# SkyworkAI/Vitron

Measured on NVIDIA H100. Metric: Vicuna-7B generated tokens/s, batch-8 x (256 vision + 512 text) prefill + 128-token greedy decode, incl. ViT-L/14 encode, higher is better.
Workload: dtype bf16

## Files before the change

### include/vitron_b200.h

```cpp
#ifndef VITRON_B200_H_
#define VITRON_B200_H_

#include <stddef.h>
#include <stdint.h>

#ifdef __cplusplus
extern "C" {
#endif

#ifndef __CUDA_RUNTIME_H__
typedef struct CUstream_st* cudaStream_t;
#endif

#define VB_ACT_NONE 0
#define VB_ACT_GELU 1
#define VB_ACT_QUICK_GELU 2
#define VB_ACT_RELU 3
#define VB_ACT_SILU 4

#define VB_GLU_NONE 0
#define VB_GLU_SWIGLU 1
#define VB_GLU_GEGLU 2

typedef struct vb_epilogue {
  const void* bias;
  const void* rowbias;
  int64_t rowbias_rows;
  const void* residual;
  int64_t ldr;
  float alpha;
  int32_t act;
  int32_t glu;
  int32_t out_fp32;
  const float* rowscale;
  float rms_eps;
} vb_epilogue;

const char* vb200_version(void);
const char* vb200_last_error(void);
int vb200_device_ok(void);
int vb200_set_pdl(int enable);
int vb200_set_attention_impl(int impl);
int vb200_attention_watchdog(uint32_t* out3);
int vb200_attention_tc_occupancy(int head_dim);

size_t vb200_gemm_bf16_workspace_size(int64_t M, int64_t N, int64_t K);
int vb200_gemm_bf16(const void* A, int64_t lda, const void* W, int64_t ldw, void* out, int64_t ldo,
                    int64_t M, int64_t N, int64_t K, const vb_epilogue* epi, void* workspace,
                    size_t workspace_bytes, cudaStream_t stream);

int vb200_gemm_nf4(const void* A, int64_t lda, const void* codes, const void* scales, const float* kscale, void* out,
                   int64_t ldo, int64_t M, int64_t N, int64_t K, const vb_epilogue* epi, cudaStream_t stream);
int vb200_nf4_dequant(const void* codes, const void* scales, const float* kscale, void* out, int64_t N, int64_t K,
                      cudaStream_t stream);



size_t vb200_conv_nhwc_workspace_size(int64_t nb, int64_t h, int64_t w, int64_t cin, int64_t cout, int kh, int kw,
                                      int stride, int pad_h, int pad_w);
int vb200_conv_nhwc_bf16(const void* X, const void* Wt, void* out, int64_t nb, int64_t h,
                         int64_t w, int64_t cin, int64_t cout, int kh, int kw, int stride,
                         int pad_h, int pad_w, const vb_epilogue* epi, void* workspace,
                         size_t workspace_bytes, cudaStream_t stream);
int vb200_set_gemm_impl(int impl);
int vb200_set_gemm_debug(int resident_b, int dbg);

int vb200_conv_nhwc_direct(const void* X, const void* Wt, const void* bias, void* out, int64_t nb,
                           int64_t h, int64_t w, int64_t cin, int64_t cout, int kh, int kw,
                           int stride, int pad_h, int pad_w, cudaStream_t stream);

int vb200_rmsnorm(const void* x, int64_t ldx, const void* weight, void* out, int64_t ldo,
                  int64_t rows, int64_t d, float eps, cudaStream_t stream);
int vb200_row_rstd(const void* x, int64_t ldx, float* out, int64_t rows, int64_t d, float eps,
                   cudaStream_t stream);
int vb200_layernorm(const void* x, int64_t ldx, const void* weight, const void* bias, void* out,
                    int64_t ldo, int64_t rows, int64_t d, float eps, cudaStream_t stream);
size_t vb200_groupnorm_workspace_size(int64_t n, int64_t groups, int64_t c);
int vb200_groupnorm_nhwc(const void* x, const void* weight, const void* bias, void* out, int64_t n,
                         int64_t spatial, int64_t c, int64_t groups, float eps, int act,
                         void* workspace, size_t workspace_bytes, cudaStream_t stream);

int vb200_attention(const void* q, const void* k, const void* v, void* out, int64_t B, int64_t H,
                    int64_t Sq, int64_t Skv, int64_t head_dim, int64_t q_sb, int64_t q_ss,
                    int64_t q_sh, int64_t k_sb, int64_t k_ss, int64_t k_sh, int64_t v_sb,
                    int64_t v_ss, int64_t v_sh, int64_t o_sb, int64_t o_ss, int64_t o_sh,
                    float scale, int causal, const int32_t* kv_len, const uint8_t* mask,
                    int64_t m_sb, int64_t m_sh, int64_t m_sq, cudaStream_t stream);
size_t vb200_attention_workspace_size(int64_t B, int64_t H, int64_t Sq, int64_t Skv, int64_t head_dim, int causal);
// ... 138 lines not shown
```

### vitron_b200/_lib.py

```python
import ctypes as C
import os

_HERE = os.path.dirname(os.path.abspath(__file__))
LIB_PATH = os.path.join(_HERE, "libvitron_b200.so")

ACT_NONE, ACT_GELU, ACT_QUICK_GELU, ACT_RELU, ACT_SILU = 0, 1, 2, 3, 4
GLU_NONE, GLU_SWIGLU, GLU_GEGLU = 0, 1, 2

_ERR = {-1: "VB_ERR_ARG", -2: "VB_ERR_CUDA", -3: "VB_ERR_WORKSPACE", -4: "VB_ERR_UNSUPPORTED",
        -5: "VB_ERR_DRIVER"}


class Epilogue(C.Structure):
    _fields_ = [
        ("bias", C.c_void_p), ("rowbias", C.c_void_p), ("rowbias_rows", C.c_int64),
        ("residual", C.c_void_p), ("ldr", C.c_int64), ("alpha", C.c_float),
        ("act", C.c_int32), ("glu", C.c_int32), ("out_fp32", C.c_int32),
        ("rowscale", C.c_void_p), ("rms_eps", C.c_float),
    ]


_p, _i64, _i32, _f, _sz = C.c_void_p, C.c_int64, C.c_int, C.c_float, C.c_size_t

SIGNATURES = {
    "vb200_version": (C.c_char_p, []),
    "vb200_last_error": (C.c_char_p, []),
    "vb200_device_ok": (_i32, []),
    "vb200_set_pdl": (_i32, [_i32]),
    "vb200_set_attention_impl": (_i32, [_i32]),
    "vb200_attention_watchdog": (_i32, [_p]),
    "vb200_attention_tc_occupancy": (_i32, [_i32]),
    "vb200_gemm_bf16_workspace_size": (_sz, [_i64, _i64, _i64]),
    "vb200_gemm_bf16": (_i32, [_p, _i64, _p, _i64, _p, _i64, _i64, _i64, _i64, C.POINTER(Epilogue), _p, _sz, _p]),
    "vb200_gemm_nf4": (_i32, [_p, _i64, _p, _p, _p, _p, _i64, _i64, _i64, _i64, C.POINTER(Epilogue), _p]),
    "vb200_nf4_dequant": (_i32, [_p, _p, _p, _p, _i64, _i64, _p]),
    "vb200_conv_nhwc_workspace_size": (_sz, [_i64, _i64, _i64, _i64, _i64, _i32, _i32, _i32, _i32, _i32]),
    "vb200_conv_nhwc_bf16": (_i32, [_p, _p, _p, _i64, _i64, _i64, _i64, _i64, _i32, _i32, _i32, _i32, _i32,
                                    C.POINTER(Epilogue), _p, _sz, _p]),
    "vb200_set_gemm_impl": (_i32, [_i32]),
    "vb200_set_gemm_debug": (_i32, [_i32, _i32]),
    "vb200_conv_nhwc_direct": (_i32, [_p, _p, _p, _p, _i64, _i64, _i64, _i64, _i64, _i32, _i32, _i32, _i32, _i32, _p]),
    "vb200_rmsnorm": (_i32, [_p, _i64, _p, _p, _i64, _i64, _i64, _f, _p]),
    "vb200_row_rstd": (_i32, [_p, _i64, _p, _i64, _i64, _f, _p]),
    "vb200_layernorm": (_i32, [_p, _i64, _p, _p, _p, _i64, _i64, _i64, _f, _p]),
    "vb200_groupnorm_workspace_size": (_sz, [_i64, _i64, _i64]),
    "vb200_groupnorm_nhwc": (_i32, [_p, _p, _p, _p, _i64, _i64, _i64, _i64, _f, _i32, _p, _sz, _p]),
    "vb200_attention": (_i32, [_p, _p, _p, _p, _i64, _i64, _i64, _i64, _i64] + [_i64] * 12 +
                        [_f, _i32, _p, _p, _i64, _i64, _i64, _p]),
    "vb200_attention_workspace_size": (_sz, [_i64, _i64, _i64, _i64, _i64, _i32]),
    "vb200_attention_ws": (_i32, [_p, _p, _p, _p, _i64, _i64, _i64, _i64, _i64] + [_i64] * 12 +
                           [_f, _i32, _p, _p, _i64, _i64, _i64, _p, _sz, _p]),
    "vb200_attention_paged_workspace_size": (_sz, [_i64, _i64, _i64, _i64, _i64]),
    "vb200_attention_paged": (_i32, [_p, _i64, _i64, _i64, _p, _p, _i64, _p, _i64, _p, _p, _p, _i64, _i64, _i64,
                                     _i64, _i64, _i64, _i64, _i64, _i64, _f, _p, _sz, _p]),
    "vb200_attention_short": (_i32, [_p, _p, _p, _p, _i64, _i64, _i64, _i64] + [_i64] * 17 + [_f, _p]),
    "vb200_add_rowgroup": (_i32, [_p, _p, _p, _i64, _i64, _i64, _i64, _p]),
    "vb200_rope_kv_append": (_i32, [_p, _i64, _p, _p, _p, _p, _p, _p, _i64, _i64, _i64, _i64, _i64, _f, _p]),
    "vb200_attn_decode_workspace_size": (_sz, [_i64, _i64, _i64, _i64]),
    "vb200_attn_decode_paged": (_i32, [_p, _i64, _p, _p, _p, _i64, _p, _p, _i64, _i64, _i64, _i64, _i64, _i64,
                                       _f, _p, _sz, _p]),
    "vb200_rope_table": (_i32, [_p, _p, _i64, _i64, _f, _p]),
    "vb200_attn_decode_rope": (_i32, [_p, _i64, _p, _p, _p, _p, _i64, _p, _p, _i64, _i64, _i64, _i64, _i64, _i64,
                                      _f, _p, _sz, _p]),
    "vb200_attn_decode_rope_beam": (_i32, [_p, _i64, _p, _p, _p, _p, _i64, _p, _p, _i64, _p, _p, _i64, _i64, _i64, _i64,
                                           _i64, _i64, _f, _p, _sz, _p]),
    "vb200_splice_multimodal": (_i32, [_p, _i64, _p, _i64, _p, _p, _i64, _i64, _p]),
    "vb200_argmax_rows": (_i32, [_p, _i32, _i64, _i64, _i64, _p, _p]),
    "vb200_argmax_advance": (_i32, [_p, _i64, _i64, _i64, _p, _p, _p, _p, _p, _i64, _p, _p]),
    "vb200_sample_advance": (_i32, [_p, _i64, _i64, _i64, _p, _p, _p, _p, _p, _p, _i64, _p, _p]),
    "vb200_beam_workspace_size": (_sz, [_i64]),
    "vb200_beam_advance": (_i32, [_p, _i64, _i64, _i64, _i64, _p, _p, _p, _p, _p, _i64, _p, _p, _p, _p, _p, _i64, _p, _p,
# ... 53 lines not shown
```

### vitron_b200/csrc/gemv.cu

```cuda
#include "common.cuh"
#include "vitron_b200.h"
#include <type_traits>

namespace vb {

struct GemvParams {
  const bf16* W; long long ldw;
  const bf16* X; long long ldx;
  void* out; long long ldo;
  int M, N, K;
  const bf16* bias; const bf16* rowbias; int rowbias_rows;
  const bf16* residual; long long ldr;
  float alpha; int act, glu, out_fp32;
  const float* rowscale; float rms_eps;
};

__device__ __forceinline__ float gemv_act(float x, int act) {
  switch (act) {
    case VB_ACT_GELU: return gelu_erf(x);
    case VB_ACT_QUICK_GELU: return quick_gelu(x);
    case VB_ACT_RELU: return fmaxf(x, 0.f);
    case VB_ACT_SILU: return silu(x);
    default: return x;
  }
}

__device__ __forceinline__ void mma16816(float (&c)[4], uint32_t a0, uint32_t a1, uint32_t a2, uint32_t a3,
                                         uint32_t b0, uint32_t b1) {
  asm("mma.sync.aligned.m16n8k16.row.col.f32.bf16.bf16.f32 {%0,%1,%2,%3}, {%4,%5,%6,%7}, {%8,%9}, {%0,%1,%2,%3};"
      : "+f"(c[0]), "+f"(c[1]), "+f"(c[2]), "+f"(c[3])
      : "r"(a0), "r"(a1), "r"(a2), "r"(a3), "r"(b0), "r"(b1));
}

__device__ __forceinline__ uint4 ldg_stream(const bf16* p, bool ok) {
  uint4 v = make_uint4(0, 0, 0, 0);
  if (ok) asm volatile("ld.global.nc.L1::no_allocate.v4.u32 {%0,%1,%2,%3}, [%4];" : "=r"(v.x), "=r"(v.y), "=r"(v.z), "=r"(v.w) : "l"(p));
  return v;
}
__device__ __forceinline__ uint4 ldg_cached(const bf16* p, bool ok) {
  uint4 v = make_uint4(0, 0, 0, 0);
  if (ok) v = __ldg(reinterpret_cast<const uint4*>(p));
  return v;
}

template <int ROWS, int NT>
__global__ void __launch_bounds__(256, 2) gemv_bf16_kernel(const GemvParams p) {
  constexpr int WARPS = 8;
  constexpr int RG = ROWS / 16;
  constexpr int KS = WARPS / RG;
  constexpr int G = 2;
  __shared__ float red[2][WARPS][16][NT * 8 + 1];
  __shared__ float red_sq[WARPS][NT * 8];
  __shared__ float rstd_s[NT * 8];

  const int warp = threadIdx.x >> 5, lane = threadIdx.x & 31;
  const int g = lane >> 2, t = lane & 3;
  const int rg = warp % RG, ks = warp / RG;
  const int ntiles = (p.N + ROWS - 1) / ROWS;
  const bf16* x0 = p.X + static_cast<long long>(min(g, p.M - 1)) * p.ldx;
  const bf16* x1 = p.X + static_cast<long long>(min(g + 8, p.M - 1)) * p.ldx;
  const bool x0ok = g < p.M, x1ok = (NT == 2) && (g + 8 < p.M);

  const int chunks = (p.K + 63) / 64;
  const int base = chunks / KS, rem = chunks % KS;
  const int c0 = ks * base + min(ks, rem);
  const int c1 = c0 + base + (ks < rem ? 1 : 0);
  const int ngroups = (c1 - c0 + G - 1) / G;
  const int npairs = (ngroups + 1) / 2;

  const bool do_rms = p.rms_eps > 0.f && p.rowscale == nullptr;
  float sq0 = 0.f, sq1 = 0.f;

  struct Buf { uint4 wl[G][2], wh[G][2]; };
  auto load_group = [&](Buf& bf, int tile, int grp) {
    const int row0 = tile * ROWS + rg * 16;
    const bf16* wa = p.W + static_cast<long long>(min(row0 + g, p.N - 1)) * p.ldw;
    const bf16* wb = p.W + static_cast<long long>(min(row0 + g + 8, p.N - 1)) * p.ldw;
    const bool live = tile < ntiles;
#pragma unroll
    for (int u = 0; u < G; ++u) {
      const int c = c0 + grp * G + u;
      const int k0 = c * 64 + 8 * t, k1 = k0 + 32;
      const bool in = live && c < c1;
      const bool ok0 = in && k0 < p.K, ok1 = in && k1 < p.K;
      bf.wl[u][0] = ldg_stream(wa + k0, ok0); bf.wl[u][1] = ldg_stream(wa + k1, ok1);
      bf.wh[u][0] = ldg_stream(wb + k0, ok0); bf.wh[u][1] = ldg_stream(wb + k1, ok1);
    }
  };
  float acc[NT][4];
  auto compute_group = [&](const Buf& bf, int grp, bool first_tile) {
    uint4 xa[G][2], xb[G][2];
#pragma unroll
    for (int u = 0; u < G; ++u) {
      const int c = c0 + grp * G + u;
      const int k0 = c * 64 + 8 * t, k1 = k0 + 32;
      const bool in = c < c1;
      const bool ok0 = in && k0 < p.K, ok1 = in && k1 < p.K;
      xa[u][0] = ldg_cached(x0 + k0, ok0 && x0ok); xa[u][1] = ldg_cached(x0 + k1, ok1 && x0ok);
      if (NT == 2) { xb[u][0] = ldg_cached(x1 + k0, ok0 && x1ok); xb[u][1] = ldg_cached(x1 + k1, ok1 && x1ok); }
    }
#pragma unroll
    for (int u = 0; u < G; ++u) {
      const uint32_t al[8] = {bf.wl[u][0].x, bf.wl[u][0].y, bf.wl[u][0].z, bf.wl[u][0].w, bf.wl[u][1].x, bf.wl[u][1].y, bf.wl[u][1].z, bf.wl[u][1].w};
      const uint32_t ah[8] = {bf.wh[u][0].x, bf.wh[u][0].y, bf.wh[u][0].z, bf.wh[u][0].w, bf.wh[u][1].x, bf.wh[u][1].y, bf.wh[u][1].z, bf.wh[u][1].w};
      const uint32_t b0[8] = {xa[u][0].x, xa[u][0].y, xa[u][0].z, xa[u][0].w, xa[u][1].x, xa[u][1].y, xa[u][1].z, xa[u][1].w};
      uint32_t b1[8] = {0, 0, 0, 0, 0, 0, 0, 0};
      if (NT == 2) {
        b1[0] = xb[u][0].x; b1[1] = xb[u][0].y; b1[2] = xb[u][0].z; b1[3] = xb[u][0].w;
        b1[4] = xb[u][1].x; b1[5] = xb[u][1].y; b1[6] = xb[u][1].z; b1[7] = xb[u][1].w;
      }
      if (do_rms && first_tile && rg == 0) {
#pragma unroll
        for (int j = 0; j < 8; ++j) {
          float2 f = unpack_bf16(b0[j]);
          sq0 += f.x * f.x + f.y * f.y;
          if (NT == 2) { float2 h2 = unpack_bf16(b1[j]); sq1 += h2.x * h2.x + h2.y * h2.y; }
        }
      }
#pragma unroll
      for (int j = 0; j < 4; ++j) {
        mma16816(acc[0], al[2 * j], ah[2 * j], al[2 * j + 1], ah[2 * j + 1], b0[2 * j], b0[2 * j + 1]);
        if (NT == 2) mma16816(acc[1], al[2 * j], ah[2 * j], al[2 * j + 1], ah[2 * j + 1], b1[2 * j], b1[2 * j + 1]);
      }
    }
  };

  Buf buf0, buf1;
  pdl_trigger();
  load_group(buf0, blockIdx.x, 0);
  load_group(buf1, blockIdx.x, 1);
  pdl_wait();

  const bool glu = p.glu != VB_GLU_NONE;
  const int out_cols = glu ? ROWS / 2 : ROWS;
  const int n_out_total = glu ? p.N / 2 : p.N;
  int par = 0;
  bool first = true;
  for (int tile = blockIdx.x; tile < ntiles; tile += gridDim.x) {
#pragma unroll
    for (int i = 0; i < NT; ++i) acc[i][0] = acc[i][1] = acc[i][2] = acc[i][3] = 0.f;
    for (int pr = 0; pr < npairs; ++pr) {
      const bool last = pr + 1 == npairs;
      compute_group(buf0, 2 * pr, first);
      if (!last) load_group(buf0, tile, 2 * pr + 2); else load_group(buf0, tile + gridDim.x, 0);
      compute_group(buf1, 2 * pr + 1, first);
      if (!last) load_group(buf1, tile, 2 * pr + 3); else load_group(buf1, tile + gridDim.x, 1);
    }
#pragma unroll
    for (int i = 0; i < NT; ++i) {
      red[par][warp][g][i * 8 + 2 * t] = acc[i][0];
      red[par][warp][g][i * 8 + 2 * t + 1] = acc[i][1];
      red[par][warp][g + 8][i * 8 + 2 * t] = acc[i][2];
      red[par][warp][g + 8][i * 8 + 2 * t + 1] = acc[i][3];
    }
    if (do_rms && first) {
      sq0 += __shfl_xor_sync(0xffffffffu, sq0, 1); sq0 += __shfl_xor_sync(0xffffffffu, sq0, 2);
      if (NT == 2) { sq1 += __shfl_xor_sync(0xffffffffu, sq1, 1); sq1 += __shfl_xor_sync(0xffffffffu, sq1, 2); }
      if (t == 0) { red_sq[warp][g] = sq0; if (NT == 2) red_sq[warp][8 + g] = sq1; }
    }
    __syncthreads();
    if (do_rms && first) {
      if (threadIdx.x < NT * 8) {
        float ss = 0.f;
#pragma unroll
        for (int s2 = 0; s2 < KS; ++s2) ss += red_sq[s2 * RG][threadIdx.x];
        rstd_s[threadIdx.x] = rsqrtf(ss / p.K + p.rms_eps);
      }
      __syncthreads();
    }
    for (int item = threadIdx.x; item < p.M * out_cols; item += 256) {
      const int tok = item / out_cols, j = item % out_cols;
      const int fa = j, fb = j + 16;
      const int na = tile * ROWS + fa;
      const int oc = glu ? tile * (ROWS / 2) + j : na;
      if (oc >= n_out_total) continue;
      float va = 0.f, vb_ = 0.f;
#pragma unroll
      for (int s2 = 0; s2 < KS; ++s2) {
        va += red[par][s2 * RG + fa / 16][fa % 16][tok];
        if (glu) vb_ += red[par][s2 * RG + (fb / 16) % RG][fb % 16][tok];
      }
      if (do_rms) { const float rs = rstd_s[tok]; va *= rs; vb_ *= rs; }
      else if (p.rowscale) { const float rs = p.rowscale[tok]; va *= rs; vb_ *= rs; }
      if (p.bias) {
        va += __bfloat162float(p.bias[na]);
        if (glu) vb_ += __bfloat162float(p.bias[na + 16]);
      }
      if (p.rowbias) {
        const bf16* rbp = p.rowbias + (tok / p.rowbias_rows) * static_cast<long long>(p.N);
        va += __bfloat162float(rbp[na]);
        if (glu) vb_ += __bfloat162float(rbp[na + 16]);
      }
      float r;
      if (p.glu == VB_GLU_SWIGLU) r = silu(va) * vb_;
      else if (p.glu == VB_GLU_GEGLU) r = va * gelu_erf(vb_);
      else r = gemv_act(va, p.act);
      if (p.residual) r = __bfloat162float(p.residual[tok * p.ldr + oc]) + p.alpha * r;
      else r *= p.alpha;
      if (p.out_fp32) reinterpret_cast<float*>(p.out)[tok * p.ldo + oc] = r;
      else reinterpret_cast<bf16*>(p.out)[tok * p.ldo + oc] = __float2bfloat16(r);
    }
    par ^= 1;
    first = false;
  }
}

}

using namespace vb;

int vb_launch_gemv(const void* A, int64_t lda, const void* W, int64_t ldw, void* out, int64_t ldo, int64_t M,
                   int64_t N, int64_t K, const vb_epilogue* e, cudaStream_t stream) {
  GemvParams p;
  p.W = reinterpret_cast<const bf16*>(W); p.ldw = ldw;
  p.X = reinterpret_cast<const bf16*>(A); p.ldx = lda;
  p.out = out; p.ldo = ldo;
  p.M = static_cast<int>(M); p.N = static_cast<int>(N); p.K = static_cast<int>(K);
  p.bias = reinterpret_cast<const bf16*>(e->bias);
  p.rowbias = reinterpret_cast<const bf16*>(e->rowbias);
  p.rowbias_rows = e->rowbias_rows > 0 ? static_cast<int>(e->rowbias_rows) : 1;
  p.residual = reinterpret_cast<const bf16*>(e->residual); p.ldr = e->ldr;
  p.alpha = e->alpha; p.act = e->act; p.glu = e->glu; p.out_fp32 = e->out_fp32;
  p.rowscale = e->rowscale; p.rms_eps = e->rms_eps;
  const bool glu = e->glu != VB_GLU_NONE;
  const bool rows32 = glu || (N / 16 > 6LL * vb_num_sms());
  const unsigned tiles = static_cast<unsigned>((N + (rows32 ? 31 : 15)) / (rows32 ? 32 : 16));
  const unsigned cap = 2u * static_cast<unsigned>(vb_num_sms());
  const unsigned grid = tiles < cap ? tiles : cap;
  cudaError_t err;
  if (M <= 8) {
    if (rows32) err = vb_launch(gemv_bf16_kernel<32, 1>, dim3(grid), dim3(256), 0, stream, p);
    else err = vb_launch(gemv_bf16_kernel<16, 1>, dim3(grid), dim3(256), 0, stream, p);
  } else {
    if (rows32) err = vb_launch(gemv_bf16_kernel<32, 2>, dim3(grid), dim3(256), 0, stream, p);
    else err = vb_launch(gemv_bf16_kernel<16, 2>, dim3(grid), dim3(256), 0, stream, p);
  }
  if (err != cudaSuccess) { vb_set_last_error(err); return VB_ERR_CUDA; }
  return VB_OK;
}
```

### vitron_b200/csrc/llm.cu

```cuda
#include "common.cuh"
#include <cstdlib>
#include "vitron_b200.h"
#include <limits.h>

namespace vb {

__global__ void rope_kv_append_kernel(bf16* __restrict__ qkv, long long ld, const int32_t* __restrict__ positions,
                                      const int32_t* __restrict__ batch_of_token,
                                      const int32_t* __restrict__ slot_of_token, bf16* __restrict__ k_pages,
                                      bf16* __restrict__ v_pages, const int32_t* __restrict__ block_table,
                                      int max_pages, int H, int hd, int page_size, float log2_theta) {
  const long long tok = blockIdx.x;
  const int half = hd / 2;
  const int chunks = half / 8;
  const int pos = positions[tok];
  const int slot = slot_of_token ? slot_of_token[tok] : pos;
  const int b = batch_of_token ? batch_of_token[tok] : 0;
  bf16* row = qkv + tok * ld;
  long long cache_off = -1;
  if (slot >= 0 && k_pages != nullptr && slot / page_size < max_pages) {
    const int page = block_table[static_cast<long long>(b) * max_pages + slot / page_size];
    cache_off = (static_cast<long long>(page) * H) * page_size * hd + static_cast<long long>(slot % page_size) * hd;
  }
  for (int item = threadIdx.x; item < H * chunks; item += blockDim.x) {
// ... 47 lines not shown
    const float4 c = __ldg(c4 + j), s = __ldg(s4 + j);
    cs[4 * j] = c.x; cs[4 * j + 1] = c.y; cs[4 * j + 2] = c.z; cs[4 * j + 3] = c.w;
    sn[4 * j] = s.x; sn[4 * j + 1] = s.y; sn[4 * j + 2] = s.z; sn[4 * j + 3] = s.w;
  }
#pragma unroll
  for (int j = 0; j < 16; ++j) {
    const float partner = __shfl_xor_sync(0xffffffffu, x[j], 4);
    const float r = (sub < 4) ? x[j] * cs[j] - partner * sn[j] : x[j] * cs[j] + partner * sn[j];
    x[j] = __bfloat162float(__float2bfloat16(r));
  }
}

__global__ void rope_table_kernel(const int32_t* __restrict__ positions, float* __restrict__ table, int half,
                                  float log2_theta) {
  const int b = blockIdx.x, i = threadIdx.x;
  pdl_trigger();
  pdl_wait();
  if (i >= half) return;
  const float inv_freq = exp2f(-(static_cast<float>(i) / half) * log2_theta);
  float sn, cs;
  sincosf(static_cast<float>(positions[b]) * inv_freq, &sn, &cs);
  table[b * 2 * half + i] = cs;
  table[b * 2 * half + half + i] = sn;
}

template <bool ROPE, int MAX_TRIPS, bool BEAM = false>
__global__ void __launch_bounds__(DEC_THREADS, 4)
attn_decode_kernel(const bf16* __restrict__ q, long long ld_q, bf16* __restrict__ k_pages,
                   bf16* __restrict__ v_pages, const int32_t* __restrict__ block_table, int max_pages,
                   const int32_t* __restrict__ kv_len, int H, int page_size, float scale, int splits, int per,
                   float* __restrict__ ws_ml, float* __restrict__ ws_o, int* __restrict__ counters,
                   bf16* __restrict__ out, long long ld_o, const float* __restrict__ rope_table,
                   const int32_t* __restrict__ beam_src, int src_ld, const int32_t* __restrict__ gen_start) {
  constexpr int HD = 128;
  const int split = blockIdx.x, h = blockIdx.y, b = blockIdx.z;
  const int warp = threadIdx.x >> 5, lane = threadIdx.x & 31;
  const int grp = lane >> 3, sub = lane & 7;
  const int32_t* bt = block_table + static_cast<long long>(b) * max_pages;
  const int c0 = split * per;
  int pg[MAX_TRIPS];
#pragma unroll
  for (int i = 0; i < MAX_TRIPS; ++i) {
    const int pi = c0 / 64 + i;
    pg[i] = (pi < max_pages && i * 64 < per) ? bt[pi] : 0;
  }
  const long long pf_head = static_cast<long long>(h) * page_size * HD;
  const long long pf_stride = static_cast<long long>(H) * page_size * HD;
  auto prefetch_page = [&](int page) {
    const long long base = static_cast<long long>(page) * pf_stride + pf_head + static_cast<long long>(threadIdx.x) * 64;
    asm volatile("prefetch.global.L2 [%0];" ::"l"(k_pages + base));
    asm volatile("prefetch.global.L2 [%0];" ::"l"(v_pages + base));
  };
  if (per > 0) prefetch_page(pg[0]);
  if (MAX_TRIPS > 1 && per > 64) prefetch_page(pg[1]);
  pdl_wait();
  pdl_trigger();
  const int len = kv_len[b];
  const int c1 = min(len, c0 + per);
  const int gstart = BEAM ? gen_start[b] : 0;

  float qv[16];
  {
    const bf16* qp = q + static_cast<long long>(b) * ld_q + h * HD + sub * 16;
    uint4 u0 = *reinterpret_cast<const uint4*>(qp), u1 = *reinterpret_cast<const uint4*>(qp + 8);
    const uint32_t uu[8] = {u0.x, u0.y, u0.z, u0.w, u1.x, u1.y, u1.z, u1.w};
#pragma unroll
    for (int j = 0; j < 8; ++j) { float2 f = unpack_bf16(uu[j]); qv[2 * j] = f.x; qv[2 * j + 1] = f.y; }
  }
  if (ROPE) {
    const float* cs_table = rope_table + b * HD;
    rope16(qv, sub, cs_table);
    const int tnew = len - 1;
    if (tnew >= c0 && tnew < c1) {
      if (warp == 0) {
        float kv_[16];
        const bf16* kp = q + static_cast<long long>(b) * ld_q + (static_cast<long long>(H) + h) * HD + sub * 16;
        uint4 u0 = *reinterpret_cast<const uint4*>(kp), u1 = *reinterpret_cast<const uint4*>(kp + 8);
        const uint32_t uu[8] = {u0.x, u0.y, u0.z, u0.w, u1.x, u1.y, u1.z, u1.w};
#pragma unroll
        for (int j = 0; j < 8; ++j) { float2 f = unpack_bf16(uu[j]); kv_[2 * j] = f.x; kv_[2 * j + 1] = f.y; }
        rope16(kv_, sub, cs_table);
        if (grp == 0) {
          const long long off = static_cast<long long>(bt[tnew / page_size]) * H * page_size * HD +
                                static_cast<long long>(h) * page_size * HD + static_cast<long long>(tnew % page_size) * HD + sub * 16;
          uint32_t w[8];
#pragma unroll
          for (int j = 0; j < 8; ++j) w[j] = pack_bf16(kv_[2 * j], kv_[2 * j + 1]);
          *reinterpret_cast<uint4*>(k_pages + off) = make_uint4(w[0], w[1], w[2], w[3]);
          *reinterpret_cast<uint4*>(k_pages + off + 8) = make_uint4(w[4], w[5], w[6], w[7]);
          const bf16* vp = q + static_cast<long long>(b) * ld_q + (2LL * H + h) * HD + sub * 16;
          *reinterpret_cast<uint4*>(v_pages + off) = *reinterpret_cast<const uint4*>(vp);
          *reinterpret_cast<uint4*>(v_pages + off + 8) = *reinterpret_cast<const uint4*>(vp + 8);
        }
      }
      __threadfence_block();
      __syncthreads();
    }
  }
#pragma unroll
  for (int j = 0; j < 16; ++j) qv[j] *= scale;
  float m = -INFINITY, l = 0.f, o[16];
#pragma unroll
  for (int j = 0; j < 16; ++j) o[j] = 0.f;
  const long long head_off = static_cast<long long>(h) * page_size * HD + sub * 16;
  const long long page_stride = static_cast<long long>(H) * page_size * HD;

  const int gid = warp * 4 + grp;
// ... 22 lines not shown
  };
  auto compute_half = [&](int hs, const Half& h) {
    float sc[2];
#pragma unroll
    for (int u = 0; u < 2; ++u) {
      const uint32_t kw[8] = {h.k[u][0].x, h.k[u][0].y, h.k[u][0].z, h.k[u][0].w, h.k[u][1].x, h.k[u][1].y, h.k[u][1].z, h.k[u][1].w};
      float a = 0.f;
#pragma unroll
      for (int j = 0; j < 8; ++j) {
        float2 f = unpack_bf16(kw[j]);
        a += qv[2 * j] * f.x + qv[2 * j + 1] * f.y;
      }
      sc[u] = a;
    }
#pragma unroll
    for (int sh = 1; sh < 8; sh <<= 1) {
#pragma unroll
      for (int u = 0; u < 2; ++u) sc[u] += __shfl_xor_sync(0xffffffffu, sc[u], sh);
    }
    float mn = m;
#pragma unroll
    for (int u = 0; u < 2; ++u) {
      const bool has = c0 + 64 * (hs >> 1) + gid + 16 * u + 32 * (hs & 1) < c1;
      if (!has) sc[u] = -INFINITY;
      mn = fmaxf(mn, sc[u]);
    }
    const float msafe = (mn == -INFINITY) ? 0.f : mn;
    const float corr = __expf(m - msafe);
    float pr[2];
    float psum = 0.f;
#pragma unroll
    for (int u = 0; u < 2; ++u) { pr[u] = __expf(sc[u] - msafe); psum += pr[u]; }
    l = l * corr + psum;
    m = mn;
#pragma unroll
    for (int j = 0; j < 16; ++j) o[j] *= corr;
#pragma unroll
    for (int u = 0; u < 2; ++u) {
      const uint32_t vw[8] = {h.v[u][0].x, h.v[u][0].y, h.v[u][0].z, h.v[u][0].w, h.v[u][1].x, h.v[u][1].y, h.v[u][1].z, h.v[u][1].w};
#pragma unroll
      for (int j = 0; j < 8; ++j) {
        float2 f = unpack_bf16(vw[j]);
        o[2 * j] += pr[u] * f.x;
        o[2 * j + 1] += pr[u] * f.y;
      }
    }
  };
  Half buf0, buf1;
  if (nh > 0) load_half(0, buf0);
#pragma unroll
  for (int hs = 0; hs < 2 * MAX_TRIPS; hs += 2) {
    if (hs >= nh) break;
    if (hs + 1 < nh) load_half(hs + 1, buf1);
    if ((hs >> 1) + 2 < MAX_TRIPS && c0 + 64 * ((hs >> 1) + 2) < c1) prefetch_page(pg[(hs >> 1) + 2]);
    compute_half(hs, buf0);
    if (hs + 1 >= nh) break;
    if (hs + 2 < nh && hs + 2 < 2 * MAX_TRIPS) load_half(hs + 2, buf0);
    compute_half(hs + 1, buf1);
  }

  __shared__ float sm_m[16], sm_l[16];
  __shared__ float sm_o[16][HD + 4];
  if (sub == 0) { sm_m[gid] = m; sm_l[gid] = l; }
#pragma unroll
  for (int j = 0; j < 16; ++j) sm_o[gid][sub * 16 + j] = o[j];
  __syncthreads();
  const int d = threadIdx.x;
  float M = -INFINITY;
#pragma unroll
  for (int g = 0; g < 16; ++g) M = fmaxf(M, sm_m[g]);
  float L = 0.f, O = 0.f;
#pragma unroll
  for (int g = 0; g < 16; ++g) {
    const float w = (sm_m[g] == -INFINITY) ? 0.f : __expf(sm_m[g] - M);
    L += sm_l[g] * w;
    O += sm_o[g][d] * w;
  }
  if (splits == 1) {
    out[static_cast<long long>(b) * ld_o + h * HD + d] = __float2bfloat16(L > 0.f ? O / L : 0.f);
  } else {
    const long long base = (static_cast<long long>(b) * H + h) * splits;
    const long long idx = base + split;
    if (d == 0) { ws_ml[idx * 2] = M; ws_ml[idx * 2 + 1] = L; }
    ws_o[idx * HD + d] = O;
    __shared__ int is_last;
    __threadfence();
    __syncthreads();
    if (d == 0) is_last = (atomicAdd(&counters[b * H + h], 1) == splits - 1) ? 1 : 0;
    __syncthreads();
    if (is_last) {
      __threadfence();
      float Mx = -INFINITY;
      for (int s = 0; s < splits; ++s) Mx = fmaxf(Mx, __ldcg(&ws_ml[(base + s) * 2]));
      float Ls = 0.f, Os = 0.f;
      for (int s = 0; s < splits; ++s) {
        const float ms = __ldcg(&ws_ml[(base + s) * 2]);
        const float w = (ms == -INFINITY) ? 0.f : __expf(ms - Mx);
        Ls += __ldcg(&ws_ml[(base + s) * 2 + 1]) * w;
        Os += __ldcg(&ws_o[(base + s) * HD + d]) * w;
      }
      out[static_cast<long long>(b) * ld_o + h * HD + d] = __float2bfloat16(Ls > 0.f ? Os / Ls : 0.f);
      if (d == 0) counters[b * H + h] = 0;
    }
  }
}

__global__ void splice_kernel(const bf16* __restrict__ embed, long long vocab, const bf16* __restrict__ feats,
// ... 799 lines not shown
```

### vitron_b200/llama.py

```python
from dataclasses import dataclass

import torch

from . import nf4 as _nf4
from . import beam as _beam
from . import ops, sampling

BF16 = torch.bfloat16


@dataclass
class LlamaConfig:
    hidden_size: int = 4096
    intermediate_size: int = 11008
    num_hidden_layers: int = 32
    num_attention_heads: int = 32
    vocab_size: int = 32000
    rms_norm_eps: float = 1e-5
    rope_theta: float = 10000.0
    max_position_embeddings: int = 4096

    @property
    def head_dim(self):
        return self.hidden_size // self.num_attention_heads
# ... 216 lines not shown
        d, f = c.hidden_size, c.intermediate_size
        gains = getattr(self, "norm_gains", None)
        ones = torch.ones((d,), dtype=torch.float32, device=self.device)
        nf4 = self.nf4

        def unfold(w, g):
            if isinstance(w, _nf4.NF4Weight):
                return _nf4.dequantize(w).to(BF16)
            return (w.float() / g[None, :]).to(BF16)
        out[prefix + "model.embed_tokens.weight"] = self.embed
        gn = gains["norm"] if gains else ones
        out[prefix + "model.norm.weight"] = gn.to(BF16)
        out[prefix + "lm_head.weight"] = unfold(self.lm_head, gn)
        for i, L in enumerate(self.layers):
            p = f"{prefix}model.layers.{i}."
            g1 = gains["ln1"][i] if gains else ones
            g2 = gains["ln2"][i] if gains else ones
            q, k, v = (L["wqkv"].rows(j * d, (j + 1) * d) for j in range(3)) if nf4 else L["wqkv"].split(d, 0)
            out[p + "self_attn.q_proj.weight"], out[p + "self_attn.k_proj.weight"], out[p + "self_attn.v_proj.weight"] = \
                unfold(q, g1), unfold(k, g1), unfold(v, g1)
            dense = lambda w: _nf4.dequantize(w).to(BF16) if nf4 else w
            out[p + "self_attn.o_proj.weight"] = dense(L["wo"])
            wgu = _nf4.dequantize(L["wgu"]) if nf4 else L["wgu"]
            gu = wgu.view(f // 16, 2, 16, d)
            out[p + "mlp.gate_proj.weight"] = unfold(gu[:, 0].reshape(f, d), ones if nf4 else g2)
            out[p + "mlp.up_proj.weight"] = unfold(gu[:, 1].reshape(f, d), ones if nf4 else g2)
            out[p + "mlp.down_proj.weight"] = dense(L["wdown"])
            out[p + "input_layernorm.weight"] = g1.to(BF16)
            out[p + "post_attention_layernorm.weight"] = g2.to(BF16)
        return out

    def parameters(self):
        yield self.embed
        yield self.lm_head
        for L in self.layers:
            for w in (L["wqkv"], L["wo"], L["wgu"], L["wdown"]):
                if isinstance(w, _nf4.NF4Weight):
                    yield from (w.codes, w.scales)
                else:
                    yield w

    def weight_bytes(self):
        n = 2 * self.lm_head.numel()
        for l in self.layers:
            for w in (l["wqkv"], l["wo"], l["wgu"], l["wdown"]):
                n += w.nbytes if isinstance(w, _nf4.NF4Weight) else 2 * w.numel()
        return n

    def _layer(self, i, h, positions, bot, slots, prefill_shape=None, kv_len=None, max_kv_len=0, q_start=None,
               beam=False):
        c, L, cache = self.cfg, self.layers[i], self.cache
        H, D = c.num_attention_heads, c.head_dim
        g1, g2 = L.get("g1"), L.get("g2")
        qkv = ops.gemm(h, L["wqkv"], rms_eps=c.rms_norm_eps, **({} if g1 is None else dict(kscale=g1)))
        if prefill_shape is not None:
            B, S = prefill_shape
            ops.rope_kv_append(qkv, positions, H, D, c.rope_theta, cache.k(i), cache.v(i), cache.block_table, bot, slots,
                               cache.page_size)
            q4 = qkv.view(B, S, 3, H, D)
            if q_start is None:
                att = ops.attention(q4[:, :, 0], q4[:, :, 1], q4[:, :, 2], causal=True, kv_len=kv_len)
            else:
                att = ops.attention_paged(q4[:, :, 0], cache.k(i), cache.v(i), cache.block_table[:B], q_start, kv_len,
                                          max_kv_len)
            att = att.view(B * S, H * D)
        elif beam:
            T = h.shape[0]
            att = ops.attn_decode_rope_beam(qkv, self._rope_tab, cache.k(i), cache.v(i), cache.block_table, kv_len,
                                            self.beam["beam_src"][:T], self.d_prompt[:T], H, D, cache.page_size,
                                            max_kv_len)
        else:
            att = ops.attn_decode_rope(qkv, self._rope_tab, cache.k(i), cache.v(i), cache.block_table, kv_len, H, D,
                                       cache.page_size, max_kv_len)
        ops.gemm(att, L["wo"], residual=h, out=h)
        act = ops.gemm(h, L["wgu"], glu=ops.GLU_SWIGLU, rms_eps=c.rms_norm_eps, **({} if g2 is None else dict(kscale=g2)))
        ops.gemm(act, L["wdown"], residual=h, out=h)
        return h

    def prefill(self, inputs_embeds, seq_lens=None, all_logits=False):
        c, dev, cache = self.cfg, self.device, self.cache
        B, S, d = inputs_embeds.shape
        if B > self.max_batch:
            raise ValueError(f"batch {B} > engine max_batch {self.max_batch}")
        lens = [S] * B if seq_lens is None else [int(x) for x in seq_lens]
        if max(lens) > cache.max_seq_len or S > cache.max_seq_len:
            raise ValueError(f"prompt of {max(max(lens), S)} tokens exceeds the KV cache capacity {cache.max_seq_len} "
                             f"(construct the model with a larger max_seq_len)")
        for b in range(self.max_batch):
            cache.release(b)
        for b in range(B):
            cache.reserve(b, lens[b])
        cache.sync_table()
        ar = torch.arange(S, dtype=torch.int32)
        lens_t = torch.tensor(lens, dtype=torch.int32)
        pos_h = ar.repeat(B)
        valid = (ar[None, :] < lens_t[:, None]).reshape(-1)
        slots_h = torch.where(valid, pos_h, torch.full_like(pos_h, -1))
        bot_h = torch.arange(B, dtype=torch.int32).repeat_interleave(S)
        positions = pos_h.to(dev, non_blocking=True)
        slots = slots_h.to(dev, non_blocking=True)
        bot = bot_h.to(dev, non_blocking=True)
        kv_len = lens_t.to(dev, non_blocking=True)
        h = inputs_embeds.to(BF16).reshape(B * S, d).clone()
        for i in range(c.num_hidden_layers):
            self._layer(i, h, positions, bot, slots, prefill_shape=(B, S), kv_len=kv_len)
        self.d_pos[:B].copy_(kv_len)
        self.d_len[:B].copy_(kv_len + 1)
        self.d_prompt[:B].copy_(kv_len)
        self._lens_host = list(lens)
        if all_logits:
            return ops.gemm(h, self.lm_head, out_fp32=True, rms_eps=c.rms_norm_eps).view(B, S, c.vocab_size)
        last = (torch.arange(B) * S + (lens_t.long() - 1)).to(dev)
        hl = h.index_select(0, last)
        return ops.gemm(hl, self.lm_head, out_fp32=True, rms_eps=c.rms_norm_eps)

    def append(self, inputs_embeds, chunk_lens, all_logits=True, past_lens=None):
        c, dev, cache = self.cfg, self.device, self.cache
        B, S, d = inputs_embeds.shape
        if B > self.max_batch:
            raise ValueError(f"batch {B} > engine max_batch {self.max_batch}")
        past = list(self._lens_host[:B]) if past_lens is None else [int(x) for x in past_lens]
        lens = [int(x) for x in chunk_lens]
        if len(past) != B or len(lens) != B or min(lens) < 1 or max(lens) > S or min(past) < 0:
            raise ValueError(f"chunk lengths {lens} / past lengths {past} do not fit a [{B}, {S}] chunk")
        total = [p + n for p, n in zip(past, lens)]
        if max(total) > cache.max_seq_len:
            raise ValueError(f"prompt of {max(total)} tokens exceeds the KV cache capacity {cache.max_seq_len} "
                             f"(construct the model with a larger max_seq_len)")
        changed = False
        for b in range(B):
            changed |= cache.reserve(b, total[b])
        if changed:
            cache.sync_table()
        ar = torch.arange(S, dtype=torch.int32)
        past_t, lens_t = torch.tensor(past, dtype=torch.int32), torch.tensor(lens, dtype=torch.int32)
        pos_h = (past_t[:, None] + ar[None, :]).reshape(-1)
        valid = (ar[None, :] < lens_t[:, None]).reshape(-1)
        slots_h = torch.where(valid, pos_h, torch.full_like(pos_h, -1))
        bot_h = torch.arange(B, dtype=torch.int32).repeat_interleave(S)
        positions, slots, bot = (t.to(dev, non_blocking=True) for t in (pos_h, slots_h, bot_h))
        q_start, q_len = past_t.to(dev, non_blocking=True), lens_t.to(dev, non_blocking=True)
        h = inputs_embeds.to(BF16).reshape(B * S, d).clone()
        for i in range(c.num_hidden_layers):
            self._layer(i, h, positions, bot, slots, prefill_shape=(B, S), kv_len=q_len, max_kv_len=max(total),
                        q_start=q_start)
        tot_t = torch.tensor(total, dtype=torch.int32).to(dev, non_blocking=True)
        self.d_pos[:B].copy_(tot_t)
        self.d_len[:B].copy_(tot_t + 1)
        self.d_prompt[:B].copy_(tot_t)
        self._lens_host = list(total)
        if all_logits:
            return ops.gemm(h, self.lm_head, out_fp32=True, rms_eps=c.rms_norm_eps).view(B, S, c.vocab_size)
        last = (torch.arange(B) * S + (lens_t.long() - 1)).to(dev)
        return ops.gemm(h.index_select(0, last), self.lm_head, out_fp32=True, rms_eps=c.rms_norm_eps)

    def _decode_body(self, B, beam=False):
        c = self.cfg
        h = ops.splice_multimodal(self.embed, None, self.d_src[:B])
        self._rope_tab = ops.rope_table(self.d_pos[:B], c.head_dim, c.rope_theta, out=self.d_rope[:B])
        for i in range(c.num_hidden_layers):
            self._layer(i, h, self.d_pos[:B], self.d_bot[:B], None, kv_len=self.d_len[:B],
                        max_kv_len=self.cache.max_seq_len, beam=beam)
        ops.gemm(h, self.lm_head, out=self.d_logits[:B], out_fp32=True, rms_eps=c.rms_norm_eps)

    def _step_kernels(self, B, sampled=False):
        from . import _lib
        lib = _lib.load()
        prev = lib.vb200_set_pdl(1 if self.use_pdl else 0)
        try:
            self._step_kernels_inner(B, sampled)
        finally:
            lib.vb200_set_pdl(prev)

    def _step_kernels_inner(self, B, sampled=False):
        if sampled == "beam":
            self._decode_body(B, beam=True)
            self.beam_advance(self.d_logits[:B])
            return
        self._decode_body(B)
        state = dict(next_src=self.d_src[:B], positions=self.d_pos[:B], kv_len=self.d_len[:B], token_log=self.token_log[:B],
                     prompt_len=self.d_prompt[:B])
        if sampled:
            self.sample_advance(self.d_logits[:B], self.d_next[:B], **state)
        else:
            ops.argmax_advance(self.d_logits[:B], self.d_next[:B], **state)

    def sample_advance(self, logits, out_idx=None, **state):
        fn = ops.sample_advance if self.device.type == "cuda" else sampling.sample_advance
        return fn(logits, self.d_sample, out_idx, **state)

    def set_sampling(self, temperature=1.0, top_k=None, top_p=None, seed=0):
        k = 0 if not top_k or top_k < 0 else min(int(top_k), 2 ** 31 - 1)
        p = 1.0 if top_p is None else float(top_p)
        self.d_sample.copy_(ops.sample_params(max(float(temperature), 1e-6), k, p, seed))

    def _beam_state(self):
        if self.beam is None:
            R, S, dev = self.max_batch, self.cache.max_seq_len, self.device
            z = lambda *shape, dt=torch.int32: torch.zeros(shape, dtype=dt, device=dev)
            self.beam = dict(beam_score=z(R, dt=torch.float32), parent=z(R), done=z(R), beam_src=z(R, S),
                             hyp_score=z(R, dt=torch.float64), hyp_len=z(R), hyp_seq=z(R), hyp_count=z(R),
                             hyp_ids=z(R, S, dt=torch.int64))
            self.d_beam = torch.zeros((_beam.PARAMS.size,), dtype=torch.uint8, device=dev)
            if dev.type == "cuda":
                ops.reserve_beam_workspace(R, dev)
        return self.beam

    def _require_beam(self):
        if self.beam is None or self.beam_k < 1:
            raise RuntimeError("no beam search is set up on this engine: call start_beam() before beam steps")

    def beam_advance(self, logits):
        self._require_beam()
        R = logits.shape[0]
        fn = ops.beam_advance if self.device.type == "cuda" else _beam.beam_advance
        fn(logits, self.beam_k, self.d_beam, **{n: t[:R] for n, t in self.beam.items()}, next_src=self.d_src[:R],
# ... 93 lines not shown
```

### vitron_b200/ops.py

```python
import ctypes as C
import math
import struct

import torch

from . import _lib, beam
from .nf4 import NF4Weight
from ._lib import (ACT_GELU, ACT_NONE, ACT_QUICK_GELU, ACT_RELU, ACT_SILU, GLU_GEGLU, GLU_NONE,
                   GLU_SWIGLU, Epilogue, check)

BF16 = torch.bfloat16
_ws = {}
_launches = [0]


def launch_count():
    return _launches[0]


def count_launches(n):
    _launches[0] += int(n)


def _stream():
# ... 41 lines not shown

    def __init__(self, fn, warmup=2):
        self.fn, self.warmup, self.graphs = fn, warmup, {}

    def __call__(self, **tensors):
        key = tuple((k, tuple(v.shape), v.dtype, v.device.index) for k, v in sorted(tensors.items()))
        ent = self.graphs.get(key)
        if ent is None:
            static = {k: v.detach().clone() for k, v in tensors.items()}
            dev = next(iter(static.values())).device
            s = torch.cuda.Stream(device=dev)
            s.wait_stream(torch.cuda.current_stream())
            with torch.cuda.stream(s):
                for _ in range(self.warmup):
                    self.fn(**static)
            torch.cuda.current_stream().wait_stream(s)
            torch.cuda.synchronize()
            g = torch.cuda.CUDAGraph()
            l0 = launch_count()
            with torch.cuda.graph(g), pdl(True):
                out = self.fn(**static)
            ent = (g, static, out, launch_count() - l0)
            self.graphs[key] = ent
        g, static, out, n = ent
        for k, v in tensors.items():
            static[k].copy_(v, non_blocking=True)
        g.replay()
        count_launches(n)
        return out


def _req(cond, msg):
    if not cond:
        raise ValueError(msg)


def _rows2d(x):
    _req(x.stride(-1) == 1, "inner dimension must be contiguous")
    if x.dim() == 2:
        return x, x.stride(0)
    x2 = x.reshape(-1, x.shape[-1])
    return x2, x2.stride(0)


def pack_glu_weight(w_a, w_b):
    f = w_a.shape[0]
    _req(f % 16 == 0 and w_a.shape == w_b.shape, "GLU halves must match and be multiples of 16 rows")
    rest = w_a.shape[1:]
    a = w_a.reshape(f // 16, 16, *rest)
    b = w_b.reshape(f // 16, 16, *rest)
    return torch.stack([a, b], dim=1).reshape(2 * f, *rest).contiguous()


def gemm(a, w, bias=None, act=ACT_NONE, glu=GLU_NONE, residual=None, alpha=1.0, rowbias=None,
         rowbias_rows=0, out=None, out_fp32=False, rowscale=None, rms_eps=0.0, kscale=None):
    lib = _lib.load()
    a2, lda = _rows2d(a)
    q4 = isinstance(w, NF4Weight)
    _req(a2.dtype == BF16 and (q4 or w.dtype == BF16), "gemm operands must be bf16 (or an NF4Weight)")
    _req(len(w.shape) == 2 and w.shape[1] == a2.shape[1] and (q4 or w.stride(1) == 1), "weight must be [N, K] row-major")
    _req(kscale is None or (q4 and kscale.dtype == torch.float32 and kscale.is_contiguous()
                            and kscale.numel() == a2.shape[1]), "kscale: fp32 [K], NF4 weights only")
    M, K = a2.shape
    N = w.shape[0]
    small = M <= (NF4_MAX_M if q4 else 16)
    n_out = N // 2 if glu != GLU_NONE else N
    if out is None:
        out = torch.empty((M, n_out), dtype=torch.float32 if out_fp32 else BF16, device=a.device)
    else:
        _req(out.shape[-1] == n_out and out.stride(-1) == 1, "bad out shape")
        _req(out.dtype == (torch.float32 if out_fp32 else BF16), "bad out dtype")
    out2, ldo = _rows2d(out)
    epi = Epilogue()
    epi.bias = _ptr(bias)
    epi.rowbias = _ptr(rowbias)
    epi.rowbias_rows = int(rowbias_rows)
    epi.alpha = float(alpha)
    epi.act = int(act)
    epi.glu = int(glu)
    epi.out_fp32 = 1 if out_fp32 else 0
    if rowscale is not None:
        _req(rowscale.dtype == torch.float32 and rowscale.numel() == M and rowscale.is_contiguous(), "bad rowscale")
        epi.rowscale = rowscale.data_ptr()
    elif rms_eps > 0:
        if small:
            epi.rms_eps = float(rms_eps)
        else:
            rs = row_rstd(a2, rms_eps)
            epi.rowscale = rs.data_ptr()
    if residual is not None:
        r2, ldr = _rows2d(residual)
        _req(r2.dtype == BF16 and r2.shape == (M, n_out), "bad residual")
        epi.residual = r2.data_ptr()
        epi.ldr = ldr
    if bias is not None:
        _req(bias.dtype == BF16 and bias.numel() == N and bias.is_contiguous(), "bad bias")
    if M == 0:
        return out.reshape(*a.shape[:-1], n_out) if a.dim() != 2 else out
    if q4 and small:
        check(lib.vb200_gemm_nf4(a2.data_ptr(), lda, w.codes.data_ptr(), w.scales.data_ptr(), _ptr(kscale),
                                 out2.data_ptr(), ldo, M, N, K, C.byref(epi), _stream()), "vb200_gemm_nf4")
        _launches[0] += 1
        return out.reshape(*a.shape[:-1], n_out) if a.dim() != 2 else out
    if q4:
        w = nf4_dequant(w, kscale, workspace(2 * N * K, a.device, "nf4"))
    need = lib.vb200_gemm_bf16_workspace_size(M, N, K)
    ws = workspace(need, a.device) if need else None
    check(lib.vb200_gemm_bf16(a2.data_ptr(), lda, w.data_ptr(), w.stride(0), out2.data_ptr(), ldo, M, N, K,
                              C.byref(epi), _ptr(ws), need, _stream()), "vb200_gemm_bf16")
    _launches[0] += 1
    return out.reshape(*a.shape[:-1], n_out) if a.dim() != 2 else out


NF4_MAX_M = 32


def nf4_dequant(w, kscale=None, out=None):
    N, K = w.shape
    if out is None:
        out = torch.empty((N, K), dtype=BF16, device=w.device)
    else:
        _req(out.is_contiguous() and out.numel() * out.element_size() >= 2 * N * K, "nf4_dequant: out too small")
        out = out.view(torch.uint8)[:2 * N * K].view(BF16).view(N, K) if out.dtype != BF16 else out.view(N, K)
    _req(kscale is None or (kscale.dtype == torch.float32 and kscale.is_contiguous() and kscale.numel() == K), "bad kscale")
    check(_lib.load().vb200_nf4_dequant(w.codes.data_ptr(), w.scales.data_ptr(), _ptr(kscale), out.data_ptr(), N, K,
                                        _stream()), "vb200_nf4_dequant")
    _launches[0] += 1
    return out


def reserve_nf4_workspace(weights, device):
    need = max((2 * w.shape[0] * w.shape[1] for w in weights), default=0)
    return workspace(need, torch.device(device), "nf4") if need else None


def set_gemm_impl(impl):
    return _lib.load().vb200_set_gemm_impl(int(impl))


def set_gemm_debug(resident_b=-1, dbg=-1):
    return _lib.load().vb200_set_gemm_debug(int(resident_b), int(dbg))


def pack_conv_weight(w):
    if w.dim() == 5:
        w = w[:, :, :, 0, 0].unsqueeze(-1)
    cout, cin, kh, kw = w.shape
    cpad = (cin + 63) // 64 * 64
    out = torch.zeros((cout, kh * kw, cpad), dtype=BF16, device=w.device)
# ... 579 lines not shown
```

Measured before the change: 1031.

## Prefetch head of next decode GEMM's weights into L2 during GEMV tail

Adds an l2_next pointer and byte count to the GEMM epilogue. During the last tile of the small-M GEMV, blocks issue L2 prefetches for the first 8 MiB of the next layer's weight matrix (o→gate/up, gate/up→down, down→next qkv, lm_head→layer0 qkv). The aim is to hide DRAM latency at kernel boundaries in memory-bound decode. The prefetch of additional KV pages in paged decode attention is also removed, likely to free bandwidth for the weight prefetch. Risks: extra DRAM traffic competing with the current GEMV, and L2 pollution.

```diff
diff --git a/include/vitron_b200.h b/include/vitron_b200.h
--- a/include/vitron_b200.h
+++ b/include/vitron_b200.h
@@ -34,6 +34,8 @@
   int32_t out_fp32;
   const float* rowscale;
   float rms_eps;
+  const void* l2_next;
+  int64_t l2_next_bytes;
 } vb_epilogue;
 
 const char* vb200_version(void);
diff --git a/vitron_b200/_lib.py b/vitron_b200/_lib.py
--- a/vitron_b200/_lib.py
+++ b/vitron_b200/_lib.py
@@ -17,6 +17,7 @@
         ("residual", C.c_void_p), ("ldr", C.c_int64), ("alpha", C.c_float),
         ("act", C.c_int32), ("glu", C.c_int32), ("out_fp32", C.c_int32),
         ("rowscale", C.c_void_p), ("rms_eps", C.c_float),
+        ("l2_next", C.c_void_p), ("l2_next_bytes", C.c_int64),
     ]
 
 
diff --git a/vitron_b200/csrc/gemv.cu b/vitron_b200/csrc/gemv.cu
--- a/vitron_b200/csrc/gemv.cu
+++ b/vitron_b200/csrc/gemv.cu
@@ -13,6 +13,7 @@
   const bf16* residual; long long ldr;
   float alpha; int act, glu, out_fp32;
   const float* rowscale; float rms_eps;
+  const char* l2_next; long long l2_next_bytes;
 };
 
 __device__ __forceinline__ float gemv_act(float x, int act) {
@@ -41,6 +42,14 @@
   uint4 v = make_uint4(0, 0, 0, 0);
   if (ok) v = __ldg(reinterpret_cast<const uint4*>(p));
   return v;
+}
+
+__device__ __forceinline__ void l2_prefetch_slice(const char* base, long long n) {
+  const long long lines = (n + 127) >> 7;
+  const long long per = (lines + gridDim.x - 1) / gridDim.x;
+  const long long lo = static_cast<long long>(blockIdx.x) * per;
+  const long long hi = min(lo + per, lines);
+  for (long long l = lo + threadIdx.x; l < hi; l += blockDim.x) asm volatile("prefetch.global.L2 [%0];" ::"l"(base + (l << 7)));
 }
 
 template <int ROWS, int NT>
@@ -139,8 +148,10 @@
   for (int tile = blockIdx.x; tile < ntiles; tile += gridDim.x) {
 #pragma unroll
     for (int i = 0; i < NT; ++i) acc[i][0] = acc[i][1] = acc[i][2] = acc[i][3] = 0.f;
+    const bool last_tile = tile + gridDim.x >= ntiles;
     for (int pr = 0; pr < npairs; ++pr) {
       const bool last = pr + 1 == npairs;
+      if (last && last_tile && p.l2_next != nullptr) l2_prefetch_slice(p.l2_next, p.l2_next_bytes);
       compute_group(buf0, 2 * pr, first);
       if (!last) load_group(buf0, tile, 2 * pr + 2); else load_group(buf0, tile + gridDim.x, 0);
       compute_group(buf1, 2 * pr + 1, first);
@@ -222,6 +233,8 @@
   p.residual = reinterpret_cast<const bf16*>(e->residual); p.ldr = e->ldr;
   p.alpha = e->alpha; p.act = e->act; p.glu = e->glu; p.out_fp32 = e->out_fp32;
   p.rowscale = e->rowscale; p.rms_eps = e->rms_eps;
+  p.l2_next = e->l2_next_bytes > 0 ? reinterpret_cast<const char*>(e->l2_next) : nullptr;
+  p.l2_next_bytes = e->l2_next_bytes;
   const bool glu = e->glu != VB_GLU_NONE;
   const bool rows32 = glu || (N / 16 > 6LL * vb_num_sms());
   const unsigned tiles = static_cast<unsigned>((N + (rows32 ? 31 : 15)) / (rows32 ? 32 : 16));
diff --git a/vitron_b200/csrc/llm.cu b/vitron_b200/csrc/llm.cu
--- a/vitron_b200/csrc/llm.cu
+++ b/vitron_b200/csrc/llm.cu
@@ -123,7 +123,6 @@
     asm volatile("prefetch.global.L2 [%0];" ::"l"(v_pages + base));
   };
   if (per > 0) prefetch_page(pg[0]);
-  if (MAX_TRIPS > 1 && per > 64) prefetch_page(pg[1]);
   pdl_wait();
   pdl_trigger();
   const int len = kv_len[b];
@@ -252,7 +251,6 @@
   for (int hs = 0; hs < 2 * MAX_TRIPS; hs += 2) {
     if (hs >= nh) break;
     if (hs + 1 < nh) load_half(hs + 1, buf1);
-    if ((hs >> 1) + 2 < MAX_TRIPS && c0 + 64 * ((hs >> 1) + 2) < c1) prefetch_page(pg[(hs >> 1) + 2]);
     compute_half(hs, buf0);
     if (hs + 1 >= nh) break;
     if (hs + 2 < nh && hs + 2 < 2 * MAX_TRIPS) load_half(hs + 2, buf0);
diff --git a/vitron_b200/llama.py b/vitron_b200/llama.py
--- a/vitron_b200/llama.py
+++ b/vitron_b200/llama.py
@@ -292,6 +292,10 @@
         c, L, cache = self.cfg, self.layers[i], self.cache
         H, D = c.num_attention_heads, c.head_dim
         g1, g2 = L.get("g1"), L.get("g2")
+        nxt = {} if prefill_shape is not None or self.device.type != "cuda" else dict(
+            o=L["wgu"], gu=L["wdown"],
+            down=self.layers[i + 1]["wqkv"] if i + 1 < c.num_hidden_layers else self.lm_head)
+        hint = lambda k: dict(l2_next=nxt[k]) if isinstance(nxt.get(k), torch.Tensor) else {}
         qkv = ops.gemm(h, L["wqkv"], rms_eps=c.rms_norm_eps, **({} if g1 is None else dict(kscale=g1)))
         if prefill_shape is not None:
             B, S = prefill_shape
@@ -312,9 +316,10 @@
         else:
             att = ops.attn_decode_rope(qkv, self._rope_tab, cache.k(i), cache.v(i), cache.block_table, kv_len, H, D,
                                        cache.page_size, max_kv_len)
-        ops.gemm(att, L["wo"], residual=h, out=h)
-        act = ops.gemm(h, L["wgu"], glu=ops.GLU_SWIGLU, rms_eps=c.rms_norm_eps, **({} if g2 is None else dict(kscale=g2)))
-        ops.gemm(act, L["wdown"], residual=h, out=h)
+        ops.gemm(att, L["wo"], residual=h, out=h, **hint("o"))
+        act = ops.gemm(h, L["wgu"], glu=ops.GLU_SWIGLU, rms_eps=c.rms_norm_eps,
+                       **({} if g2 is None else dict(kscale=g2)), **hint("gu"))
+        ops.gemm(act, L["wdown"], residual=h, out=h, **hint("down"))
         return h
 
     def prefill(self, inputs_embeds, seq_lens=None, all_logits=False):
@@ -401,7 +406,9 @@
         for i in range(c.num_hidden_layers):
             self._layer(i, h, self.d_pos[:B], self.d_bot[:B], None, kv_len=self.d_len[:B],
                         max_kv_len=self.cache.max_seq_len, beam=beam)
-        ops.gemm(h, self.lm_head, out=self.d_logits[:B], out_fp32=True, rms_eps=c.rms_norm_eps)
+        w0 = self.layers[0]["wqkv"]
+        ops.gemm(h, self.lm_head, out=self.d_logits[:B], out_fp32=True, rms_eps=c.rms_norm_eps,
+                 **(dict(l2_next=w0) if self.device.type == "cuda" and isinstance(w0, torch.Tensor) else {}))
 
     def _step_kernels(self, B, sampled=False):
         from . import _lib
diff --git a/vitron_b200/ops.py b/vitron_b200/ops.py
--- a/vitron_b200/ops.py
+++ b/vitron_b200/ops.py
@@ -117,8 +117,11 @@
     return torch.stack([a, b], dim=1).reshape(2 * f, *rest).contiguous()
 
 
+L2_NEXT_BYTES = 8 << 20
+
+
 def gemm(a, w, bias=None, act=ACT_NONE, glu=GLU_NONE, residual=None, alpha=1.0, rowbias=None,
-         rowbias_rows=0, out=None, out_fp32=False, rowscale=None, rms_eps=0.0, kscale=None):
+         rowbias_rows=0, out=None, out_fp32=False, rowscale=None, rms_eps=0.0, kscale=None, l2_next=None):
     lib = _lib.load()
     a2, lda = _rows2d(a)
     q4 = isinstance(w, NF4Weight)
@@ -160,6 +163,10 @@
         epi.ldr = ldr
     if bias is not None:
         _req(bias.dtype == BF16 and bias.numel() == N and bias.is_contiguous(), "bad bias")
+    if l2_next is not None and L2_NEXT_BYTES > 0:
+        _req(l2_next.is_contiguous() and l2_next.device == a.device, "l2_next must be a contiguous tensor on a's device")
+        epi.l2_next = l2_next.data_ptr()
+        epi.l2_next_bytes = min(L2_NEXT_BYTES, l2_next.numel() * l2_next.element_size())
     if M == 0:
         return out.reshape(*a.shape[:-1], n_out) if a.dim() != 2 else out
     if q4 and small:
```

Result: faster. 1080, median of 6 (+4.8%).
